# mbrzus/Cross-Modality-Minipig-Gan

Hardware: NVIDIA B200
Metric: gan_train_image_pairs_per_sec (higher is better)
Workload: dtype bf16

## Files before the change

### cross-modality-minipig-gan_b200/csrc/conv_c1mma.cuh

```cuda
#pragma once

namespace mpgan {
namespace tc {

constexpr int kC1Threads = 512;
constexpr int kC1XStages = 16;
constexpr int kC1XBytes = 2304;
constexpr int kC1Stages = 8;
constexpr int kC1StageBytes = 128 * 32;

struct C1mmaParams {
  int nimg, ih, iw, oh, ow, stride, pad;
  int tiles_w, tiles_h, total_tiles;
  int xrow;
  uint32_t xbytes;
  int xoff;
  int wide;
  const bf16* w;
  bf16* out;
  long long out_sn, out_sh, out_sw;
  const float* bias;
  double* stats;
};

template <int N>
__global__ void __launch_bounds__(kC1Threads, 1)
c1mma_fprop_kernel(const __grid_constant__ C1mmaParams P, const __grid_constant__ CUtensorMap tmX) {
  constexpr int NACC = 512 / N > 8 ? 8 : 512 / N;
  constexpr int TMEM_COLS = NACC * N < 32 ? 32 : NACC * N;
  constexpr int CH = N >= 32 ? 32 : 16;
  constexpr int NCH = N / CH;
  constexpr uint32_t kEmptyArrivals = NCH == 1 ? 4u : 8u;
  extern __shared__ __align__(1024) uint8_t smem[];
  if ((smem_u32(smem) & 1023u) != 0) __trap();
  uint8_t* a_sm = smem;
  uint8_t* x_sm = smem + kC1Stages * kC1StageBytes;
  uint8_t* w_sm = x_sm + kC1XStages * kC1XBytes;
  uint64_t* a_full = reinterpret_cast<uint64_t*>(w_sm + 2048);
  uint64_t* a_empty = a_full + kC1Stages;
  uint64_t* tfull = a_empty + kC1Stages;
  uint64_t* tempty = tfull + 8;
  uint64_t* x_full = tempty + 8;
  uint64_t* x_empty = x_full + kC1XStages;
  uint32_t* tmem_slot = reinterpret_cast<uint32_t*>(x_empty + kC1XStages);
  float* s_stats = reinterpret_cast<float*>(w_sm + 2048 + 1024);
  float* s_bias = s_stats + 8 * 2 * N;

  const int warp = threadIdx.x >> 5, lane = threadIdx.x & 31;
  if (threadIdx.x == 0) {
    for (int i = 0; i < kC1Stages; ++i) { mbar_init(&a_full[i], 1); mbar_init(&a_empty[i], 1); }
    for (int i = 0; i < 8; ++i) { mbar_init(&tfull[i], 1); mbar_init(&tempty[i], kEmptyArrivals); }
    for (int i = 0; i < kC1XStages; ++i) { mbar_init(&x_full[i], 1); mbar_init(&x_empty[i], 1); }
    fence_barrier_init();
    prefetch_tmap(&tmX);
  }
  if (warp == 4) tmem_alloc<TMEM_COLS>(tmem_slot);
  for (int i = threadIdx.x; i < 8 * 2 * N; i += blockDim.x) s_stats[i] = 0.f;
  pdl_wait();
  pdl_launch();
  if (threadIdx.x < N) {
    const int n = threadIdx.x;
    uint32_t v[8];
#pragma unroll
    for (int j = 0; j < 8; ++j) v[j] = 0u;
#pragma unroll
    for (int t = 0; t < 9; ++t) {
      const uint32_t b = (uint32_t)__bfloat16_as_ushort(P.w[n * 9 + t]);
      v[t >> 1] |= (t & 1) ? (b << 16) : b;
    }
    const uint32_t sw = (uint32_t)(n >> 2) & 1u;
    *reinterpret_cast<uint4*>(w_sm + n * 32 + ((0u ^ sw) << 4)) = make_uint4(v[0], v[1], v[2], v[3]);
    *reinterpret_cast<uint4*>(w_sm + n * 32 + ((1u ^ sw) << 4)) = make_uint4(v[4], v[5], v[6], v[7]);
    s_bias[n] = P.bias ? __ldg(&P.bias[n]) : 0.f;
    asm volatile("fence.proxy.async.shared::cta;" ::: "memory");
  }
  tc_fence_before();
  __syncthreads();
  tc_fence_after();
  const uint32_t tmem_base = *tmem_slot;
  const int tiles_per_img = P.tiles_w * P.tiles_h;

  if (warp == 5) {
    if (elect_one()) {
      int xs = 0;
      uint32_t xpar = 0;
      TileWalk<3> tw;
      { const int radix[3] = {P.tiles_w, P.tiles_h, 1 << 30}; tw.init((int)blockIdx.x, (int)gridDim.x, radix); }
      for (int tile = blockIdx.x; tile < P.total_tiles; tile += gridDim.x, tw.next()) {
        const int twi = tw.d[0], thi = tw.d[1], img = tw.d[2];
        mbar_wait(&x_empty[xs], xpar ^ 1);
        mbar_expect_tx(&x_full[xs], P.xbytes);
        tma_load_3d(x_sm + xs * kC1XBytes, &tmX, &x_full[xs], twi * HT_W * P.stride - P.pad - P.xoff,
                    thi * HT_H * P.stride - P.pad, img);
        if (++xs == kC1XStages) { xs = 0; xpar ^= 1; }
      }
    }
  } else if (warp < 4) {
    const int S = P.stride;
    int it = warp;
    for (int tile = blockIdx.x + warp * gridDim.x; tile < P.total_tiles; tile += 4 * gridDim.x, it += 4) {
      const int stage = it % kC1Stages;
      const uint32_t par = (uint32_t)(it / kC1Stages) & 1u;
      const int xs = it % kC1XStages;
      const uint32_t xpar = (uint32_t)(it / kC1XStages) & 1u;
      mbar_wait(&x_full[xs], xpar);
      const uint8_t* xw = x_sm + xs * kC1XBytes;
      uint32_t v[4][9];
#pragma unroll
      for (int k = 0; k < 4; ++k) {
// ... 54 lines not shown
    for (int j = 0; j < CH / 2; ++j) { s1[j] = 0ull; s2[j] = 0ull; }
    int it = 0;
    TileWalk<3> tw;
    { const int radix[3] = {P.tiles_w, P.tiles_h, 1 << 30}; tw.init((int)blockIdx.x, (int)gridDim.x, radix); }
    for (int tile = blockIdx.x; tile < P.total_tiles; tile += gridDim.x, ++it, tw.next()) {
      if (NCH == 1 && (it & 1) != half) continue;
      const int twi = tw.d[0], thi = tw.d[1], img = tw.d[2];
      const int oh = thi * HT_H + lh, ow = twi * HT_W + lw;
      const bool valid = oh < P.oh && ow < P.ow;
      bf16* orow = P.out + (long long)img * P.out_sn + (long long)oh * P.out_sh + (long long)ow * P.out_sw + c0;
      const int acc = it % NACC;
      const uint32_t par = (uint32_t)(it / NACC) & 1u;
      mbar_wait(&tfull[acc], par);
      tc_fence_after();
      const uint32_t t_addr = tmem_base + ((uint32_t)(q * 32) << 16) + (uint32_t)(acc * N + c0);
      uint32_t r[CH];
      if (CH == 32) tmem_ld_32x32(t_addr, r);
      else tmem_ld_32x16(t_addr, r);
      tmem_ld_wait();
      tc_fence_before();
      __syncwarp();
      if (lane == 0) mbar_arrive(&tempty[acc]);
      epi_chunk_store<CH>(r, s_bias + c0, orow, valid, P.stats != nullptr, s1, s2, nullptr, P.wide != 0);
    }
    if (P.stats) {
      float v[32];
#pragma unroll
      for (int j = 0; j < 32; ++j) v[j] = j < CH ? ((j & 1) ? unpack_f32x2(s1[j / 2]).y : unpack_f32x2(s1[j / 2]).x) : 0.f;
      const float t1 = warp_transpose_reduce32(v, lane);
#pragma unroll
      for (int j = 0; j < 32; ++j) v[j] = j < CH ? ((j & 1) ? unpack_f32x2(s2[j / 2]).y : unpack_f32x2(s2[j / 2]).x) : 0.f;
      const float t2 = warp_transpose_reduce32(v, lane);
      if (lane < CH) { sl[c0 + lane] = t1; sl[N + c0 + lane] = t2; }
    }
  }
  __syncwarp();
  tc_fence_before();
  __syncthreads();
  if (P.stats) {
    for (int i = threadIdx.x; i < 2 * N; i += blockDim.x) {
      double s = 0.0;
#pragma unroll
      for (int e = 0; e < 8; ++e) s += (double)s_stats[e * 2 * N + i];
      if (s != 0.0) atomicAdd(&P.stats[i], s);
    }
  }
  if (warp == 4) {
    tc_fence_after();
    tmem_dealloc<TMEM_COLS>(tmem_base);
  }
}

template <int N>
static int launch_c1mma(const C1mmaParams& P, const CUtensorMap& mX, cudaStream_t s) {
  const size_t smem = (size_t)kC1Stages * kC1StageBytes + (size_t)kC1XStages * kC1XBytes + 2048 + 1024 +
                      (size_t)8 * 2 * N * 4 + (size_t)N * 4 + 64;
  static bool attr_done = false;
  if (!attr_done) {
    cudaError_t e = cudaFuncSetAttribute(c1mma_fprop_kernel<N>, cudaFuncAttributeMaxDynamicSharedMemorySize, 96 * 1024);
    MPGAN_REQUIRE(e == cudaSuccess, MPGAN_ERR_CUDA, "cudaFuncSetAttribute(c1mma): %s", cudaGetErrorString(e));
    attr_done = true;
  }
  const int grid = P.total_tiles < num_sms() ? P.total_tiles : num_sms();
  launch_k(c1mma_fprop_kernel<N>, grid, kC1Threads, smem, s, P, mX);
  MPGAN_CHECK_LAUNCH("c1mma_fprop_kernel");
  return 0;
}

}

int c1mma_fprop(const MpganConvGeom* g, int dtype, const void* x, int64_t ldx, const void* w, const float* bias, void* y,
                int64_t ldy, double* stats, cudaStream_t s) {
  using namespace tc;
  if (!g || dtype != MPGAN_BF16 || g->rank != 2 || g->cx != 1) return 1;
  if (g->k[1] != 3 || g->k[2] != 3 || g->stride[1] != g->stride[2] || (g->stride[1] != 1 && g->stride[1] != 2)) return 1;
  if (g->pad[1] != g->pad[2] || g->pad[1] < 0 || g->pad[1] > 1) return 1;
  if (g->stride[1] != 1) return 1;
  const int N = g->cy;
  if (!(N == 16 || N == 32 || N == 64)) return 1;
  if (ldy % 8 != 0 || ((uintptr_t)y & 15) || ((uintptr_t)x & 15)) return 1;
  if (ldx != 1 || g->xs[2] % 8 != 0) return 1;
  C1mmaParams P;
  memset(&P, 0, sizeof(P));
  P.nimg = g->n; P.ih = g->xs[1]; P.iw = g->xs[2]; P.oh = g->ys[1]; P.ow = g->ys[2];
  P.stride = g->stride[1]; P.pad = g->pad[1];
  P.tiles_w = (P.ow + HT_W - 1) / HT_W; P.tiles_h = (P.oh + HT_H - 1) / HT_H;
  P.total_tiles = g->n * P.tiles_w * P.tiles_h;
  P.w = (const bf16*)w;
  P.xoff = P.pad ? 8 - P.pad : 0;
  const int need = (HT_W - 1) * P.stride + 3 + P.xoff;
  const int bw = need <= 16 ? 16 : 32, bh = (HT_H - 1) * P.stride + 3;
  P.xrow = bw * 2; P.xbytes = (uint32_t)(bw * 2 * bh);
  if ((int)P.xbytes > kC1XBytes) return 1;
  CUtensorMap mX;
  {
    uint64_t dims[3] = {(uint64_t)P.iw, (uint64_t)P.ih, (uint64_t)g->n};
    uint64_t str[2] = {(uint64_t)P.iw, (uint64_t)P.iw * P.ih};
    uint32_t box[3] = {(uint32_t)bw, (uint32_t)bh, 1u};
    int rc = encode_map(&mX, x, 3, dims, str, box, true);
    if (rc) return rc;
  }
  P.out = (bf16*)y;
  P.out_sn = (long long)P.oh * P.ow * ldy; P.out_sh = (long long)P.ow * ldy; P.out_sw = ldy;
  P.bias = bias; P.stats = stats;
  P.wide = (ldy % 16 == 0 && ((uintptr_t)y & 31) == 0) ? 1 : 0;
  switch (N) {
    case 16: return launch_c1mma<16>(P, mX, s);
    case 32: return launch_c1mma<32>(P, mX, s);
    default: return launch_c1mma<64>(P, mX, s);
  }
}

}
```

### cross-modality-minipig-gan_b200/csrc/conv_tc.cu

```cuda
#include <cudaTypedefs.h>
#include <algorithm>
#include <stdlib.h>
#include <string.h>

#include "common.cuh"
#include "tc_common.cuh"

namespace mpgan {
namespace tc {

constexpr int MAXT = 64;
constexpr int MAXCLS = 8;
constexpr int kSmemLimit = 227 * 1024;

struct ActMaps { CUtensorMap m[8]; };

struct TapGemmParams {
  int ncls;
  int cls_tap_begin[MAXCLS + 1];
  int cls_od[MAXCLS], cls_oh[MAXCLS], cls_ow[MAXCLS];
  long long cls_out_off[MAXCLS];
  signed char tap_map[MAXT];
  short tap_dd[MAXT], tap_dh[MAXT], tap_dw[MAXT], tap_slab[MAXT];
  int nkc;
// ... 1137 lines not shown
}

extern "C" size_t mpgan_tc_conv_wgrad_workspace(const MpganConvGeom* g) {
  (void)g;
  return 0;
}

extern "C" int mpgan_tc_conv_wgrad(const MpganConvGeom* g, const void* x, int64_t ldx, const void* y, int64_t ldy,
                                   float* dw, void* workspace, size_t workspace_bytes, void* stream) {
  (void)workspace; (void)workspace_bytes;
  Geom2 g2;
  int rc = to_geom2(g, &g2);
  if (rc) return rc;
  return run_wgrad(g2, x, ldx, y, ldy, dw, (cudaStream_t)stream);
}
```

### cross-modality-minipig-gan_b200/mpgan/_lib.py

```python
import ctypes
import os
import re
from ctypes import c_char_p, c_double, c_float, c_int, c_int32, c_int64, c_size_t, c_void_p, POINTER, Structure

_HERE = os.path.dirname(os.path.abspath(__file__))
LIB_PATH = os.path.join(os.path.dirname(_HERE), "libmpgan_sm100.so")
HEADER_PATH = os.path.join(os.path.dirname(os.path.dirname(_HERE)), "include", "mpgan.h")

F32, BF16 = 0, 1
ACT_NONE, ACT_PRELU, ACT_LEAKY, ACT_TANH = 0, 1, 2, 3


class ConvGeom(Structure):
    _fields_ = [("rank", c_int32), ("n", c_int32), ("xs", c_int32 * 3), ("ys", c_int32 * 3), ("cx", c_int32),
                ("cy", c_int32), ("k", c_int32 * 3), ("stride", c_int32 * 3), ("pad", c_int32 * 3)]


_G = POINTER(ConvGeom)
_P = c_void_p
_SIGS = {
    "mpgan_version": (c_int, []),
    "mpgan_last_error": (c_char_p, []),
    "mpgan_device_ok": (c_int, []),
    "mpgan_conv_fprop": (c_int, [_G, c_int, _P, c_int64, _P, _P, _P, c_int64, _P]),
# ... 36 lines not shown
    "mpgan_bce_bwd": (c_int, [_P, _P, c_float, _P, _P, c_int32, _P]),
    "mpgan_l1_fwd": (c_int, [c_int, _P, _P, c_int64, c_float, _P, _P]),
    "mpgan_l1_bwd": (c_int, [c_int, _P, _P, c_int64, c_float, _P, _P, c_int, _P]),
    "mpgan_l1_fwd_bwd": (c_int, [c_int, _P, _P, c_int64, c_float, _P, _P, _P, _P, c_int, _P]),
    "mpgan_adam_step": (c_int, [_P, _P, _P, _P, c_int64, c_float, c_float, c_float, c_float, _P, _P, _P]),
    "mpgan_cast": (c_int, [c_int, _P, c_int, _P, c_int64, _P]),
    "mpgan_weight_transpose": (c_int, [c_int, _P, c_int, _P, c_int32, c_int32, c_int32, _P]),
    "mpgan_weight_transpose_batch": (c_int, [_P, c_int32, c_int32, _P]),
    "mpgan_patch_gather": (c_int, [c_int, _P, c_int32, c_int32, _P, c_int32, _P, c_int32, c_int32, _P, _P]),
    "mpgan_patch_scatter_add": (c_int, [c_int, _P, c_int32, c_int32, _P, c_int32, _P, c_int32, c_int32, _P, _P]),
    "mpgan_c1_tail_fwd": (c_int, [_P, c_int32, c_int32, c_int32, _P, _P, _P, c_float, c_float, _P, _P, _P, _P, _P, _P,
                                  _P, _P, _P, _P, _P, _P, _P]),
    "mpgan_c1_tail_bwd_reduce": (c_int, [_P, _P, c_int32, c_int32, c_int32, _P, _P, _P, _P, _P, _P, _P, _P, _P]),
    "mpgan_im2col_c1": (c_int, [_P, c_int32, c_int32, c_int32, c_int32, c_int32, c_int32, c_int32, _P, _P]),
    "mpgan_fold_dw16": (c_int, [_P, c_int32, _P, _P]),
    "mpgan_im2col_c1_vol": (c_int, [_P, c_int32, POINTER(c_int32), POINTER(c_int32), c_int32, c_int32, _P, _P]),
    "mpgan_col2im_c1_vol": (c_int, [_P, c_int32, POINTER(c_int32), POINTER(c_int32), c_int32, c_int32, _P, _P, _P, _P]),
    "mpgan_fold_dw32": (c_int, [_P, c_int32, _P, _P]),
    "mpgan_stencil27": (c_int, [c_int, c_int, _P, c_int32, c_int32, c_int32, c_int32, _P, _P, _P, _P, _P]),
    "mpgan_stencil27_wgrad": (c_int, [c_int, _P, _P, c_int32, c_int32, c_int32, c_int32, _P, _P, _P]),
    "mpgan_order_stats_workspace": (c_size_t, [c_int32]),
    "mpgan_order_stats": (c_int, [_P, c_int64, _P, c_int32, _P, _P, c_size_t, _P]),
    "mpgan_minmax": (c_int, [_P, c_int64, _P, c_int32, _P, _P, c_size_t, _P]),
    "mpgan_rescale_intensity": (c_int, [_P, c_int64, c_float, c_float, c_float, c_float, c_int, c_float, c_float, c_int,
                                        c_int, _P, _P]),
    "mpgan_err_sums": (c_int, [_P, _P, c_int64, _P, _P]),
    "mpgan_ssim_sums": (c_int, [_P, _P, c_int32, c_int32, c_int32, c_int32, c_int32, POINTER(c_double), c_int32, c_double,
                                c_double, c_double, _P, _P]),
    "mpgan_mutual_info_workspace": (c_size_t, [c_int32]),
    "mpgan_mutual_info": (c_int, [_P, _P, c_int32, c_int64, c_int32, _P, _P, _P, _P, c_size_t, _P]),
# ... 50 lines not shown
```

### cross-modality-minipig-gan_b200/mpgan/nets.py

```python
import os

import numpy as np
import torch
import torch.nn as nn

from . import ops
from ._lib import ACT_LEAKY, ACT_NONE, ACT_PRELU
from .runtime import Runtime

_CONV = {2: nn.Conv2d, 3: nn.Conv3d}
_CONVT = {2: nn.ConvTranspose2d, 3: nn.ConvTranspose3d}
_BN = {2: nn.BatchNorm2d, 3: nn.BatchNorm3d}

DEFAULT_PRECISION = "bf16"


def remap_monai_keys(state_dict, to="legacy"):
    out = type(state_dict)() if isinstance(state_dict, dict) else {}
    for k, v in state_dict.items():
        if to == "legacy":
            k = k.replace(".adn.N.", ".norm.").replace(".adn.A.", ".act.")
        elif "generator." in k or k.startswith("model."):
            k = k.replace(".norm.", ".adn.N.").replace(".act.", ".adn.A.")
        out[k] = v
# ... 539 lines not shown
        self._init_runtime(precision)

    def _run(self, x, save, want_acts, need_wgrad=None, logical_acts=True):
        rt = self.runtime
        rt.ensure(x.device)
        plan = Plan(rt, self.training, save, rt.requires_grad() if need_wgrad is None else need_wgrad)
        xin = self._to_cl(x.float())
        h = ops.add_copy(xin, None, _new(xin, xin.shape, rt.dtype)) if rt.dtype != torch.float32 else xin
        acts = []
        convs = [m for m in self.model_conv if isinstance(m, (nn.Conv2d, nn.Conv3d))]
        bns = [m for m in self.model_conv if isinstance(m, (nn.BatchNorm2d, nn.BatchNorm3d))]
        for conv, bn in zip(convs, bns):
            rec = rt.rec[conv]
            ch = conv.out_channels
            stats = plan.zeros64(2 * ch, x.device) if plan.training else None
            c, fused = conv_apply(rec, h, stats=stats)
            if want_acts:
                bn_out, saved = bn_act_forward(c, bn, ACT_NONE, None, 0.0, None, None, plan, stats, fused)
                y = ops.bn_act_apply(bn_out, None, None, ACT_LEAKY, None, 0.2, None, _new(c, c.shape))
                acts += [("sp", c), ("sp", bn_out), ("sp", y)]
            else:
                bn_out = None
                y, saved = bn_act_forward(c, bn, ACT_LEAKY, None, 0.2, None, None, plan, stats, fused)
            if save:
                plan.tape.append((h, c, saved, plan.training, bn_out))
            h = y
        n = h.shape[0]
        feat_shape = tuple(h.shape)
        hf = h.reshape(n, -1)
        if want_acts:
# ... 94 lines not shown
            nd = self.dims
            g = g.permute((0,) + tuple(range(2, nd + 2)) + (1,)).reshape(dfeat.shape)
            dfeat = dfeat + g.to(dfeat.dtype)
        dh = dfeat.reshape(feat_shape)
        convs = [m for m in self.model_conv if isinstance(m, (nn.Conv2d, nn.Conv3d))]
        bns = [m for m in self.model_conv if isinstance(m, (nn.BatchNorm2d, nn.BatchNorm3d))]
        nd = self.dims
        to_cl = (0,) + tuple(range(2, nd + 2)) + (1,)
        for i in range(len(convs) - 1, -1, -1):
            h_in, c, saved, trained, bn_out = plan.tape.pop()
            if (3 * i + 2) in ag:
                if internal:
                    dh = inject(dh.contiguous(), ag[3 * i + 2])
                else:
                    dh = dh + ag[3 * i + 2].permute(to_cl).to(dh.dtype)
            if bn_out is not None:
                dbn = ops.act_bwd(dh.contiguous(), bn_out, ACT_LEAKY, 0.2, _new(bn_out, bn_out.shape))
                if (3 * i + 1) in ag:
                    dbn = inject(dbn, ag[3 * i + 1]) if internal else dbn + ag[3 * i + 1].permute(to_cl).to(dbn.dtype)
                dc = bn_act_backward(dbn, c, saved, bns[i], ACT_NONE, None, 0.0, plan, trained)
                fused_bias = False
            else:
                fused_bias = (3 * i) not in ag
                dc = bn_act_backward(dh, c, saved, bns[i], ACT_LEAKY, None, 0.2, plan, trained,
                                     conv_db=rt.rec[convs[i]].db if fused_bias else None)
            if (3 * i) in ag:
                dc = inject(dc, ag[3 * i]) if internal else dc + ag[3 * i].permute(to_cl).to(dc.dtype)
            dh = conv_backward(rt.rec[convs[i]], h_in, dc, plan, need_dx=(need_dx or i > 0), bias_done=fused_bias)
            if on_layer_done is not None:
                forked = plan.wgrad_forked and N_WGRAD_STREAMS == 1
                if plan.wgrad_forked and not forked:
# ... 46 lines not shown
```

### cross-modality-minipig-gan_b200/mpgan/ops.py

```python
import bisect
import ctypes
import os

import torch

from . import _lib
from ._lib import ACT_LEAKY, ACT_NONE, ACT_PRELU, ACT_TANH, BF16, F32, ConvGeom, check

_NULL = None


def _stream():
    return torch.cuda.current_stream().cuda_stream


def dt(t):
    if t.dtype == torch.float32:
        return F32
    if t.dtype == torch.bfloat16:
        return BF16
    raise TypeError(f"unsupported dtype {t.dtype}")


def ptr(t):
# ... 266 lines not shown
        g1 = _spec_1x1(16, spec.cy).geom(n, ys, ys)
        check(lib.mpgan_tc_conv_wgrad(ctypes.byref(g1), ptr(xcol), 16, ptr(y), ld(y), ptr(dw16), None, 0, _stream()),
              "tc_conv_wgrad(im2col)")
        check(lib.mpgan_fold_dw16(ptr(dw16), spec.cy, ptr(dw), _stream()), "fold_dw16")
    elif use_tc and x.dtype == torch.bfloat16 and tc_supported(g, 2):
        check(lib.mpgan_tc_conv_wgrad(ctypes.byref(g), ptr(x), ld(x), ptr(y), ld(y), ptr(dw), None, 0, _stream()),
              "tc_conv_wgrad")
    elif use_c1 and lib.mpgan_c1_supported(ctypes.byref(g), 2):
        check(lib.mpgan_c1_conv_wgrad(ctypes.byref(g), dt(x), ptr(x), ld(x), ptr(y), ld(y), ptr(dw), _stream()),
              "c1_conv_wgrad")
    else:
        check(lib.mpgan_conv_wgrad(ctypes.byref(g), dt(x), ptr(x), ld(x), ptr(y), ld(y), ptr(dw), _stream()),
              "conv_wgrad")


def colsum(x, out):
    lib = _lib.require_device()
    check(lib.mpgan_colsum(dt(x), ptr(x), ld(x), pixels(x), x.shape[-1], ptr(out), _stream()), "colsum")


def bn_stats(x, stats):
    lib = _lib.require_device()
    check(lib.mpgan_bn_stats(dt(x), ptr(x), ld(x), pixels(x), x.shape[-1], ptr(stats), _stream()), "bn_stats")


def bn_finalize(stats, npix, bn, training, mean, invstd, scale, shift):
    lib = _lib.require_device()
    mom = 0.1 if bn.momentum is None else bn.momentum
    check(lib.mpgan_bn_finalize(ptr(stats), npix, bn.num_features, ptr(bn.weight), ptr(bn.bias), bn.eps, mom,
                                1 if training else 0, ptr(bn.running_mean), ptr(bn.running_var),
# ... 328 lines not shown
```

### include/mpgan.h

```cpp
#ifndef MPGAN_H_
#define MPGAN_H_

#include <stddef.h>
#include <stdint.h>

#ifdef __cplusplus
extern "C" {
#endif

#define MPGAN_VERSION 100

enum { MPGAN_OK = 0, MPGAN_ERR_SHAPE = -1, MPGAN_ERR_UNSUPPORTED = -2, MPGAN_ERR_CUDA = -3 };
enum { MPGAN_F32 = 0, MPGAN_BF16 = 1 };
enum { MPGAN_ACT_NONE = 0, MPGAN_ACT_PRELU = 1, MPGAN_ACT_LEAKY = 2, MPGAN_ACT_TANH = 3 };

typedef struct {
  int32_t rank;
  int32_t n;
  int32_t xs[3];
  int32_t ys[3];
  int32_t cx, cy;
  int32_t k[3], stride[3], pad[3];
} MpganConvGeom;

// ... 98 lines not shown
                            void* stream);

int mpgan_c1_tail_fwd(const void* c_bf16, int32_t n, int32_t h, int32_t w, const double* stats, const float* gamma,
                      const float* beta, float eps, float momentum, float* running_mean, float* running_var,
                      int64_t* num_batches_tracked, float* mean, float* invstd, float* scale, float* shift,
                      const float* alpha, const void* w9_bf16, const float* bias, void* h_out_bf16, void* y_out_bf16,
                      void* stream);
int mpgan_c1_tail_bwd_reduce(const void* dy_bf16, const void* c_bf16, int32_t n, int32_t h, int32_t w, const float* mean,
                             const float* invstd, const float* scale, const float* shift, const float* alpha,
                             const void* w9_bf16, void* dh_bf16, double* sums3, void* stream);

int mpgan_im2col_c1(const void* x_bf16, int32_t n, int32_t ih, int32_t iw, int32_t oh, int32_t ow, int32_t stride,
                    int32_t pad, void* xcol_bf16, void* stream);
int mpgan_fold_dw16(const float* dw16, int32_t cy, float* dw, void* stream);

int mpgan_im2col_c1_vol(const void* x_bf16, int32_t n, const int32_t* xs3, const int32_t* ys3, int32_t stride, int32_t pad,
                        void* xcol_bf16, void* stream);
int mpgan_col2im_c1_vol(const void* t_bf16, int32_t n, const int32_t* xs3, const int32_t* ys3, int32_t stride, int32_t pad,
                        const float* bias, const void* res_bf16, void* x_bf16, void* stream);
int mpgan_fold_dw32(const float* dw32, int32_t cy, float* dw, void* stream);
int mpgan_stencil27(int dtype, int direction, const void* in, int32_t n, int32_t d, int32_t h, int32_t w, const void* w27,
                    const float* bias, const void* res, void* out, void* stream);
int mpgan_stencil27_wgrad(int dtype, const void* x, const void* dy, int32_t n, int32_t d, int32_t h, int32_t w, float* dw27,
                          float* dbias, void* stream);

size_t mpgan_order_stats_workspace(int32_t nranks);
int mpgan_order_stats(const float* x, int64_t n, const int64_t* ranks, int32_t nranks, float* out, void* workspace,
                      size_t workspace_bytes, void* stream);
int mpgan_minmax(const float* x, int64_t n, const int64_t* ranks, int32_t nranks, float* out, void* workspace,
                 size_t workspace_bytes, void* stream);
// ... 23 lines not shown
```

Measured before the change: 1755.

## Fuse discriminator layer-1 conv with BatchNorm and LeakyReLU via recompute

Adds BatchNorm-aware modes to the 1-channel 3x3 tensor-core conv kernel. The forward pass runs the conv twice, once for statistics only and once applying BN plus LeakyReLU, so the large 64-channel pre-activation tensor is never written. Backward recomputes the conv, streams dy through a new TMA producer warp, and fuses the BN/activation gradient reduction and apply into two passes. This trades extra cheap conv recompute and larger shared-memory use for avoiding reads and writes of the full-resolution intermediate activations.

```diff
diff --git a/cross-modality-minipig-gan_b200/csrc/conv_c1mma.cuh b/cross-modality-minipig-gan_b200/csrc/conv_c1mma.cuh
--- a/cross-modality-minipig-gan_b200/csrc/conv_c1mma.cuh
+++ b/cross-modality-minipig-gan_b200/csrc/conv_c1mma.cuh
@@ -8,6 +8,14 @@
 constexpr int kC1XBytes = 2304;
 constexpr int kC1Stages = 8;
 constexpr int kC1StageBytes = 128 * 32;
+constexpr int kC1DyStages = 8;
+constexpr int kC1DyBytes = 128 * 64 * 2;
+
+enum { C1_CONV = 0,
+       C1_STATS = 1,
+       C1_FWD = 2,
+       C1_REDUCE = 3,
+       C1_APPLY = 4 };
 
 struct C1mmaParams {
   int nimg, ih, iw, oh, ow, stride, pad;
@@ -21,11 +29,127 @@
   long long out_sn, out_sh, out_sw;
   const float* bias;
   double* stats;
+  long long npix;
+  float slope;
+  const double* stats_in;
+  const float* gamma; const float* beta; float eps, momentum;
+  float* running_mean; float* running_var; long long* nbt;
+  float* mean; float* invstd; float* scale; float* shift;
+  float* dgamma; float* dbeta; float* dbias;
 };
 
-template <int N>
+__host__ __device__ constexpr int c1_dy_offset(int N) {
+  return (kC1Stages * kC1StageBytes + kC1XStages * kC1XBytes + 2048 + 1024 + 8 * 2 * N * 4 + N * 4 + 4 * N * 4 + 1023) &
+         ~1023;
+}
+
+template <int MODE>
+__device__ __forceinline__ void c1_bn_coef(const C1mmaParams& P, int n, int N, float* s_coef) {
+  if (MODE == C1_FWD) {
+    const double m = P.stats_in[n] / (double)P.npix;
+    double var = P.stats_in[N + n] / (double)P.npix - m * m;
+    if (var < 0.0) var = 0.0;
+    const float mean = (float)m;
+    const float invstd = (float)(1.0 / sqrt(var + (double)P.eps));
+    const float g = P.gamma ? P.gamma[n] : 1.f, b = P.beta ? P.beta[n] : 0.f;
+    const float sc = g * invstd;
+    const float sh = b - mean * sc;
+    if (blockIdx.x == 0) {
+      if (P.running_mean) P.running_mean[n] = (1.f - P.momentum) * P.running_mean[n] + P.momentum * mean;
+      if (P.running_var) {
+        const double unb = P.npix > 1 ? var * ((double)P.npix / (double)(P.npix - 1)) : var;
+        P.running_var[n] = (1.f - P.momentum) * P.running_var[n] + P.momentum * (float)unb;
+      }
+      P.mean[n] = mean; P.invstd[n] = invstd; P.scale[n] = sc; P.shift[n] = sh;
+      if (n == 0 && P.nbt) *P.nbt += 1;
+    }
+    s_coef[n] = sc; s_coef[N + n] = sh;
+  } else if (MODE == C1_REDUCE) {
+    const float sc = P.scale[n], sh = P.shift[n], mu = P.mean[n], is = P.invstd[n];
+    s_coef[n] = sc; s_coef[N + n] = sh; s_coef[2 * N + n] = is; s_coef[3 * N + n] = -mu * is;
+  } else if (MODE == C1_APPLY) {
+    const float invP = 1.f / (float)P.npix;
+    const float sc = P.scale[n], sh = P.shift[n], mu = P.mean[n], is = P.invstd[n];
+    const float mg = (float)P.stats_in[n] * invP;
+    const float mgx = (float)P.stats_in[N + n] * invP;
+    const float k2 = -sc * is * mgx;
+    s_coef[n] = sc; s_coef[N + n] = sh; s_coef[2 * N + n] = k2; s_coef[3 * N + n] = -sc * mg - k2 * mu;
+    if (blockIdx.x == 0) {
+      if (P.dbeta) P.dbeta[n] += (float)P.stats_in[n];
+      if (P.dgamma) P.dgamma[n] += (float)P.stats_in[N + n];
+    }
+  }
+}
+
+template <int MODE>
+__device__ __forceinline__ void c1_bn_epilogue(const uint32_t (&r)[16], int hh, const float* s_bias_c0, const float* s_coef_c0,
+                                               const uint8_t* dyrow, int rsw, int chunk0, bf16* orow, bool valid,
+                                               float slope, unsigned long long (&s1)[16], unsigned long long (&s2)[16]) {
+  constexpr int N = 64;
+  const unsigned long long ones = pack_f32x2(1.f, 1.f);
+  s_bias_c0 += 16 * hh; s_coef_c0 += 16 * hh; chunk0 += 2 * hh; orow += 16 * hh;
+  uint32_t o[8];
+  uint4 gq = make_uint4(0u, 0u, 0u, 0u);
+#pragma unroll
+  for (int j = 0; j < 8; ++j) {
+    const int js = 8 * hh + j;
+    if ((MODE == C1_REDUCE || MODE == C1_APPLY) && (j & 3) == 0)
+      gq = *reinterpret_cast<const uint4*>(dyrow + (((chunk0 + (j >> 2)) ^ rsw) << 4));
+    const float2 b = *reinterpret_cast<const float2*>(s_bias_c0 + 2 * j);
+    const float2 v = unpack_f32x2(fma_f32x2(pack_f32x2(__uint_as_float(r[2 * j]), __uint_as_float(r[2 * j + 1])), ones,
+                                            pack_f32x2(b.x, b.y)));
+    __nv_bfloat162 h = __floats2bfloat162_rn(v.x, v.y);
+    const uint32_t hc = *reinterpret_cast<uint32_t*>(&h);
+    const unsigned long long c = pack_f32x2(__uint_as_float(hc << 16), __uint_as_float(hc & 0xffff0000u));
+    if (MODE == C1_STATS) {
+      if (valid) {
+        s1[js] = fma_f32x2(c, ones, s1[js]);
+        s2[js] = fma_f32x2(c, c, s2[js]);
+      }
+      continue;
+    }
+    const float2 sc = *reinterpret_cast<const float2*>(s_coef_c0 + 2 * j);
+    const float2 sh = *reinterpret_cast<const float2*>(s_coef_c0 + N + 2 * j);
+    const float2 z = unpack_f32x2(fma_f32x2(c, pack_f32x2(sc.x, sc.y), pack_f32x2(sh.x, sh.y)));
+    if (MODE == C1_FWD) {
+      const float yx = z.x > 0.f ? z.x : z.x * slope, yy = z.y > 0.f ? z.y : z.y * slope;
+      __nv_bfloat162 hy = __floats2bfloat162_rn(yx, yy);
+      o[j] = *reinterpret_cast<uint32_t*>(&hy);
+      continue;
+    }
+    const float2 kc = *reinterpret_cast<const float2*>(s_coef_c0 + 2 * N + 2 * j);
+    const float2 kd = *reinterpret_cast<const float2*>(s_coef_c0 + 3 * N + 2 * j);
+    const uint32_t gw = (j & 3) == 0 ? gq.x : (j & 3) == 1 ? gq.y : (j & 3) == 2 ? gq.z : gq.w;
+    const float gx = __uint_as_float(gw << 16), gy = __uint_as_float(gw & 0xffff0000u);
+    const float2 gz = make_float2(gx * (z.x > 0.f ? 1.f : slope), gy * (z.y > 0.f ? 1.f : slope));
+    if (MODE == C1_REDUCE) {
+      const unsigned long long xh = fma_f32x2(c, pack_f32x2(kc.x, kc.y), pack_f32x2(kd.x, kd.y));
+      if (valid) {
+        const float2 a = unpack_f32x2(s1[js]);
+        s1[js] = pack_f32x2(a.x + gz.x, a.y + gz.y);
+        s2[js] = fma_f32x2(pack_f32x2(gz.x, gz.y), xh, s2[js]);
+      }
+    } else {
+      const float2 dx = unpack_f32x2(fma_f32x2(pack_f32x2(sc.x, sc.y), pack_f32x2(gz.x, gz.y),
+                                               fma_f32x2(pack_f32x2(kc.x, kc.y), c, pack_f32x2(kd.x, kd.y))));
+      __nv_bfloat162 hd = __floats2bfloat162_rn(dx.x, dx.y);
+      o[j] = *reinterpret_cast<uint32_t*>(&hd);
+      if (valid) {
+        const float2 a = unpack_f32x2(s1[js]);
+        s1[js] = pack_f32x2(a.x + __uint_as_float(o[j] << 16), a.y + __uint_as_float(o[j] & 0xffff0000u));
+      }
+    }
+  }
+  if ((MODE == C1_FWD || MODE == C1_APPLY) && valid)
+    st_global_256(orow, o[0], o[1], o[2], o[3], o[4], o[5], o[6], o[7]);
+}
+
+template <int N, int MODE>
 __global__ void __launch_bounds__(kC1Threads, 1)
-c1mma_fprop_kernel(const __grid_constant__ C1mmaParams P, const __grid_constant__ CUtensorMap tmX) {
+c1mma_fprop_kernel(const __grid_constant__ C1mmaParams P, const __grid_constant__ CUtensorMap tmX,
+                   const __grid_constant__ CUtensorMap tmDy) {
+  static_assert(MODE == C1_CONV || N == 64, "the BatchNorm modes are D layer 1 (64 channels)");
+  constexpr bool kDy = MODE == C1_REDUCE || MODE == C1_APPLY;
   constexpr int NACC = 512 / N > 8 ? 8 : 512 / N;
   constexpr int TMEM_COLS = NACC * N < 32 ? 32 : NACC * N;
   constexpr int CH = N >= 32 ? 32 : 16;
@@ -42,17 +166,24 @@
   uint64_t* tempty = tfull + 8;
   uint64_t* x_full = tempty + 8;
   uint64_t* x_empty = x_full + kC1XStages;
-  uint32_t* tmem_slot = reinterpret_cast<uint32_t*>(x_empty + kC1XStages);
+  uint64_t* dy_full = x_empty + kC1XStages;
+  uint64_t* dy_empty = dy_full + kC1DyStages;
+  uint32_t* tmem_slot = reinterpret_cast<uint32_t*>(dy_empty + kC1DyStages);
   float* s_stats = reinterpret_cast<float*>(w_sm + 2048 + 1024);
   float* s_bias = s_stats + 8 * 2 * N;
+  float* s_coef = s_bias + N;
+  uint8_t* dy_sm = smem + c1_dy_offset(N);
 
   const int warp = threadIdx.x >> 5, lane = threadIdx.x & 31;
   if (threadIdx.x == 0) {
     for (int i = 0; i < kC1Stages; ++i) { mbar_init(&a_full[i], 1); mbar_init(&a_empty[i], 1); }
     for (int i = 0; i < 8; ++i) { mbar_init(&tfull[i], 1); mbar_init(&tempty[i], kEmptyArrivals); }
     for (int i = 0; i < kC1XStages; ++i) { mbar_init(&x_full[i], 1); mbar_init(&x_empty[i], 1); }
+    if (kDy)
+      for (int i = 0; i < kC1DyStages; ++i) { mbar_init(&dy_full[i], 1); mbar_init(&dy_empty[i], 8); }
     fence_barrier_init();
     prefetch_tmap(&tmX);
+    if (kDy) prefetch_tmap(&tmDy);
   }
   if (warp == 4) tmem_alloc<TMEM_COLS>(tmem_slot);
   for (int i = threadIdx.x; i < 8 * 2 * N; i += blockDim.x) s_stats[i] = 0.f;
@@ -73,6 +204,7 @@
     *reinterpret_cast<uint4*>(w_sm + n * 32 + ((1u ^ sw) << 4)) = make_uint4(v[4], v[5], v[6], v[7]);
     s_bias[n] = P.bias ? __ldg(&P.bias[n]) : 0.f;
     asm volatile("fence.proxy.async.shared::cta;" ::: "memory");
+    if (MODE != C1_CONV && MODE != C1_STATS) c1_bn_coef<MODE>(P, n, N, s_coef);
   }
   tc_fence_before();
   __syncthreads();
@@ -93,6 +225,19 @@
         tma_load_3d(x_sm + xs * kC1XBytes, &tmX, &x_full[xs], twi * HT_W * P.stride - P.pad - P.xoff,
                     thi * HT_H * P.stride - P.pad, img);
         if (++xs == kC1XStages) { xs = 0; xpar ^= 1; }
+      }
+    }
+  } else if (warp == 6) {
+    if (kDy && elect_one()) {
+      int ds = 0;
+      uint32_t dpar = 0;
+      TileWalk<3> tw;
+      { const int radix[3] = {P.tiles_w, P.tiles_h, 1 << 30}; tw.init((int)blockIdx.x, (int)gridDim.x, radix); }
+      for (int tile = blockIdx.x; tile < P.total_tiles; tile += gridDim.x, tw.next()) {
+        mbar_wait(&dy_empty[ds], dpar ^ 1);
+        mbar_expect_tx(&dy_full[ds], (uint32_t)kC1DyBytes);
+        tma_load_4d(dy_sm + ds * kC1DyBytes, &tmDy, &dy_full[ds], 0, tw.d[0] * HT_W, tw.d[1] * HT_H, tw.d[2]);
+        if (++ds == kC1DyStages) { ds = 0; dpar ^= 1; }
       }
     }
   } else if (warp < 4) {
@@ -177,16 +322,54 @@
       mbar_wait(&tfull[acc], par);
       tc_fence_after();
       const uint32_t t_addr = tmem_base + ((uint32_t)(q * 32) << 16) + (uint32_t)(acc * N + c0);
-      uint32_t r[CH];
-      if (CH == 32) tmem_ld_32x32(t_addr, r);
-      else tmem_ld_32x16(t_addr, r);
-      tmem_ld_wait();
-      tc_fence_before();
-      __syncwarp();
-      if (lane == 0) mbar_arrive(&tempty[acc]);
-      epi_chunk_store<CH>(r, s_bias + c0, orow, valid, P.stats != nullptr, s1, s2, nullptr, P.wide != 0);
-    }
-    if (P.stats) {
+      if constexpr (MODE == C1_CONV) {
+        uint32_t r[CH];
+        if (CH == 32) tmem_ld_32x32(t_addr, r);
+        else tmem_ld_32x16(t_addr, r);
+        tmem_ld_wait();
+        tc_fence_before();
+        __syncwarp();
+        if (lane == 0) mbar_arrive(&tempty[acc]);
+        epi_chunk_store<CH>(r, s_bias + c0, orow, valid, P.stats != nullptr, s1, s2, nullptr, P.wide != 0);
+      } else {
+        const uint8_t* dyrow = nullptr;
+        int ds = 0;
+        if (kDy) {
+          ds = it % kC1DyStages;
+          mbar_wait(&dy_full[ds], (uint32_t)(it / kC1DyStages) & 1u);
+          dyrow = dy_sm + ds * kC1DyBytes + row * 128;
+        }
+#pragma unroll
+        for (int hh = 0; hh < 2; ++hh) {
+          uint32_t r[16];
+          tmem_ld_32x16(t_addr + 16 * hh, r);
+          tmem_ld_wait();
+          if (hh == 1) {
+            tc_fence_before();
+            __syncwarp();
+            if (lane == 0) mbar_arrive(&tempty[acc]);
+          }
+          c1_bn_epilogue<MODE>(r, hh, s_bias + c0, s_coef + c0, dyrow, row & 7, c0 / 8, orow, valid, P.slope, s1, s2);
+        }
+        if (kDy) {
+          __syncwarp();
+          if (lane == 0) mbar_arrive(&dy_empty[ds]);
+        }
+      }
+    }
+    if (MODE != C1_CONV && MODE != C1_FWD) {
+      float v[32];
+#pragma unroll
+      for (int j = 0; j < 32; ++j) v[j] = (j & 1) ? unpack_f32x2(s1[j / 2]).y : unpack_f32x2(s1[j / 2]).x;
+      const float t1 = warp_transpose_reduce32(v, lane);
+      float t2 = 0.f;
+      if (MODE != C1_APPLY) {
+#pragma unroll
+        for (int j = 0; j < 32; ++j) v[j] = (j & 1) ? unpack_f32x2(s2[j / 2]).y : unpack_f32x2(s2[j / 2]).x;
+        t2 = warp_transpose_reduce32(v, lane);
+      }
+      sl[c0 + lane] = t1; sl[N + c0 + lane] = t2;
+    } else if (MODE == C1_CONV && P.stats) {
       float v[32];
 #pragma unroll
       for (int j = 0; j < 32; ++j) v[j] = j < CH ? ((j & 1) ? unpack_f32x2(s1[j / 2]).y : unpack_f32x2(s1[j / 2]).x) : 0.f;
@@ -200,7 +383,15 @@
   __syncwarp();
   tc_fence_before();
   __syncthreads();
-  if (P.stats) {
+  if (MODE == C1_APPLY) {
+    if (P.dbias)
+      for (int i = threadIdx.x; i < N; i += blockDim.x) {
+        double s = 0.0;
+#pragma unroll
+        for (int e = 0; e < 8; ++e) s += (double)s_stats[e * 2 * N + i];
+        atomicAdd(&P.dbias[i], (float)s);
+      }
+  } else if (MODE != C1_FWD && P.stats) {
     for (int i = threadIdx.x; i < 2 * N; i += blockDim.x) {
       double s = 0.0;
 #pragma unroll
@@ -214,26 +405,29 @@
   }
 }
 
-template <int N>
-static int launch_c1mma(const C1mmaParams& P, const CUtensorMap& mX, cudaStream_t s) {
-  const size_t smem = (size_t)kC1Stages * kC1StageBytes + (size_t)kC1XStages * kC1XBytes + 2048 + 1024 +
-                      (size_t)8 * 2 * N * 4 + (size_t)N * 4 + 64;
+template <int N, int MODE>
+static int launch_c1mma(const C1mmaParams& P, const CUtensorMap& mX, const CUtensorMap& mDy, cudaStream_t s) {
+  size_t smem = (size_t)kC1Stages * kC1StageBytes + (size_t)kC1XStages * kC1XBytes + 2048 + 1024 +
+                (size_t)8 * 2 * N * 4 + (size_t)N * 4 + 64;
+  if (MODE != C1_CONV) smem += (size_t)4 * N * 4;
+  if (MODE == C1_REDUCE || MODE == C1_APPLY) smem = (size_t)c1_dy_offset(N) + (size_t)kC1DyStages * kC1DyBytes + 64;
   static bool attr_done = false;
   if (!attr_done) {
-    cudaError_t e = cudaFuncSetAttribute(c1mma_fprop_kernel<N>, cudaFuncAttributeMaxDynamicSharedMemorySize, 96 * 1024);
+    cudaError_t e = cudaFuncSetAttribute(c1mma_fprop_kernel<N, MODE>, cudaFuncAttributeMaxDynamicSharedMemorySize,
+                                         (int)(smem > 96 * 1024 ? kSmemLimit : 96 * 1024));
     MPGAN_REQUIRE(e == cudaSuccess, MPGAN_ERR_CUDA, "cudaFuncSetAttribute(c1mma): %s", cudaGetErrorString(e));
     attr_done = true;
   }
   const int grid = P.total_tiles < num_sms() ? P.total_tiles : num_sms();
-  launch_k(c1mma_fprop_kernel<N>, grid, kC1Threads, smem, s, P, mX);
+  launch_k(c1mma_fprop_kernel<N, MODE>, grid, kC1Threads, smem, s, P, mX, mDy);
   MPGAN_CHECK_LAUNCH("c1mma_fprop_kernel");
   return 0;
 }
 
 }
 
-int c1mma_fprop(const MpganConvGeom* g, int dtype, const void* x, int64_t ldx, const void* w, const float* bias, void* y,
-                int64_t ldy, double* stats, cudaStream_t s) {
+static int c1mma_setup(const MpganConvGeom* g, int dtype, const void* x, int64_t ldx, const void* w, const float* bias,
+                       tc::C1mmaParams* P, CUtensorMap* mX) {
   using namespace tc;
   if (!g || dtype != MPGAN_BF16 || g->rank != 2 || g->cx != 1) return 1;
   if (g->k[1] != 3 || g->k[2] != 3 || g->stride[1] != g->stride[2] || (g->stride[1] != 1 && g->stride[1] != 2)) return 1;
@@ -241,37 +435,80 @@
   if (g->stride[1] != 1) return 1;
   const int N = g->cy;
   if (!(N == 16 || N == 32 || N == 64)) return 1;
-  if (ldy % 8 != 0 || ((uintptr_t)y & 15) || ((uintptr_t)x & 15)) return 1;
+  if ((uintptr_t)x & 15) return 1;
   if (ldx != 1 || g->xs[2] % 8 != 0) return 1;
+  memset(P, 0, sizeof(*P));
+  P->nimg = g->n; P->ih = g->xs[1]; P->iw = g->xs[2]; P->oh = g->ys[1]; P->ow = g->ys[2];
+  P->stride = g->stride[1]; P->pad = g->pad[1];
+  P->tiles_w = (P->ow + HT_W - 1) / HT_W; P->tiles_h = (P->oh + HT_H - 1) / HT_H;
+  P->total_tiles = g->n * P->tiles_w * P->tiles_h;
+  P->w = (const bf16*)w;
+  P->bias = bias;
+  P->npix = (long long)g->n * P->oh * P->ow;
+  P->xoff = P->pad ? 8 - P->pad : 0;
+  const int need = (HT_W - 1) * P->stride + 3 + P->xoff;
+  const int bw = need <= 16 ? 16 : 32, bh = (HT_H - 1) * P->stride + 3;
+  P->xrow = bw * 2; P->xbytes = (uint32_t)(bw * 2 * bh);
+  if ((int)P->xbytes > kC1XBytes) return 1;
+  uint64_t dims[3] = {(uint64_t)P->iw, (uint64_t)P->ih, (uint64_t)g->n};
+  uint64_t str[2] = {(uint64_t)P->iw, (uint64_t)P->iw * P->ih};
+  uint32_t box[3] = {(uint32_t)bw, (uint32_t)bh, 1u};
+  return encode_map(mX, x, 3, dims, str, box, true);
+}
+
+int c1mma_fprop(const MpganConvGeom* g, int dtype, const void* x, int64_t ldx, const void* w, const float* bias, void* y,
+                int64_t ldy, double* stats, cudaStream_t s) {
+  using namespace tc;
   C1mmaParams P;
-  memset(&P, 0, sizeof(P));
-  P.nimg = g->n; P.ih = g->xs[1]; P.iw = g->xs[2]; P.oh = g->ys[1]; P.ow = g->ys[2];
-  P.stride = g->stride[1]; P.pad = g->pad[1];
-  P.tiles_w = (P.ow + HT_W - 1) / HT_W; P.tiles_h = (P.oh + HT_H - 1) / HT_H;
-  P.total_tiles = g->n * P.tiles_w * P.tiles_h;
-  P.w = (const bf16*)w;
-  P.xoff = P.pad ? 8 - P.pad : 0;
-  const int need = (HT_W - 1) * P.stride + 3 + P.xoff;
-  const int bw = need <= 16 ? 16 : 32, bh = (HT_H - 1) * P.stride + 3;
-  P.xrow = bw * 2; P.xbytes = (uint32_t)(bw * 2 * bh);
-  if ((int)P.xbytes > kC1XBytes) return 1;
   CUtensorMap mX;
-  {
-    uint64_t dims[3] = {(uint64_t)P.iw, (uint64_t)P.ih, (uint64_t)g->n};
-    uint64_t str[2] = {(uint64_t)P.iw, (uint64_t)P.iw * P.ih};
-    uint32_t box[3] = {(uint32_t)bw, (uint32_t)bh, 1u};
-    int rc = encode_map(&mX, x, 3, dims, str, box, true);
-    if (rc) return rc;
-  }
+  if (ldy % 8 != 0 || ((uintptr_t)y & 15)) return 1;
+  int rc = c1mma_setup(g, dtype, x, ldx, w, bias, &P, &mX);
+  if (rc) return rc;
   P.out = (bf16*)y;
   P.out_sn = (long long)P.oh * P.ow * ldy; P.out_sh = (long long)P.ow * ldy; P.out_sw = ldy;
-  P.bias = bias; P.stats = stats;
+  P.stats = stats;
   P.wide = (ldy % 16 == 0 && ((uintptr_t)y & 31) == 0) ? 1 : 0;
-  switch (N) {
-    case 16: return launch_c1mma<16>(P, mX, s);
-    case 32: return launch_c1mma<32>(P, mX, s);
-    default: return launch_c1mma<64>(P, mX, s);
-  }
-}
-
-}
+  switch (g->cy) {
+    case 16: return launch_c1mma<16, C1_CONV>(P, mX, mX, s);
+    case 32: return launch_c1mma<32, C1_CONV>(P, mX, mX, s);
+    default: return launch_c1mma<64, C1_CONV>(P, mX, mX, s);
+  }
+}
+
+static int c1bn_run(int mode, const MpganConvGeom* g, const void* x, const void* w, const float* bias, tc::C1mmaParams& P,
+                    const void* dy, void* out, cudaStream_t s) {
+  using namespace tc;
+  const tc::C1mmaParams keep = P;
+  CUtensorMap mX, mDy;
+  MPGAN_REQUIRE(g && g->cy == 64 && g->pad[1] == 0, MPGAN_ERR_UNSUPPORTED, "c1bn: 64 output channels, no padding");
+  int rc = c1mma_setup(g, MPGAN_BF16, x, 1, w, bias, &P, &mX);
+  MPGAN_REQUIRE(rc != 1, MPGAN_ERR_UNSUPPORTED, "c1bn: layer not covered by the one-channel tcgen05 kernel");
+  if (rc) return rc;
+  P.stats = keep.stats; P.slope = keep.slope; P.stats_in = keep.stats_in;
+  P.gamma = keep.gamma; P.beta = keep.beta; P.eps = keep.eps; P.momentum = keep.momentum;
+  P.running_mean = keep.running_mean; P.running_var = keep.running_var; P.nbt = keep.nbt;
+  P.mean = keep.mean; P.invstd = keep.invstd; P.scale = keep.scale; P.shift = keep.shift;
+  P.dgamma = keep.dgamma; P.dbeta = keep.dbeta; P.dbias = keep.dbias;
+  if (out) {
+    MPGAN_REQUIRE(((uintptr_t)out & 31) == 0, MPGAN_ERR_SHAPE, "c1bn: output not 32-byte aligned");
+    P.out = (bf16*)out;
+    P.out_sn = (long long)P.oh * P.ow * 64; P.out_sh = (long long)P.ow * 64; P.out_sw = 64;
+    P.wide = 1;
+  }
+  mDy = mX;
+  if (dy) {
+    uint64_t dims[4] = {64u, (uint64_t)P.ow, (uint64_t)P.oh, (uint64_t)g->n};
+    uint64_t str[3] = {64u, (uint64_t)P.ow * 64, (uint64_t)P.ow * P.oh * 64};
+    uint32_t box[4] = {64u, (uint32_t)HT_W, (uint32_t)HT_H, 1u};
+    rc = encode_map(&mDy, dy, 4, dims, str, box);
+    if (rc) return rc;
+  }
+  switch (mode) {
+    case C1_STATS: return launch_c1mma<64, C1_STATS>(P, mX, mDy, s);
+    case C1_FWD: return launch_c1mma<64, C1_FWD>(P, mX, mDy, s);
+    case C1_REDUCE: return launch_c1mma<64, C1_REDUCE>(P, mX, mDy, s);
+    default: return launch_c1mma<64, C1_APPLY>(P, mX, mDy, s);
+  }
+}
+
+}
diff --git a/cross-modality-minipig-gan_b200/csrc/conv_tc.cu b/cross-modality-minipig-gan_b200/csrc/conv_tc.cu
--- a/cross-modality-minipig-gan_b200/csrc/conv_tc.cu
+++ b/cross-modality-minipig-gan_b200/csrc/conv_tc.cu
@@ -1175,3 +1175,39 @@
   if (rc) return rc;
   return run_wgrad(g2, x, ldx, y, ldy, dw, (cudaStream_t)stream);
 }
+
+
+extern "C" int mpgan_c1bn_fwd(const MpganConvGeom* g, const void* x, const void* w, const float* bias, double* stats,
+                              const float* gamma, const float* beta, float eps, float momentum, float* running_mean,
+                              float* running_var, int64_t* num_batches_tracked, float* mean, float* invstd, float* scale,
+                              float* shift, float leaky_slope, void* y, void* stream) {
+  MPGAN_REQUIRE(stats && mean && invstd && scale && shift && y, MPGAN_ERR_SHAPE, "c1bn_fwd: bad arguments");
+  tc::C1mmaParams P;
+  memset(&P, 0, sizeof(P));
+  P.stats = stats;
+  int rc = c1bn_run(tc::C1_STATS, g, x, w, bias, P, nullptr, nullptr, (cudaStream_t)stream);
+  if (rc) return rc;
+  memset(&P, 0, sizeof(P));
+  P.stats_in = stats; P.gamma = gamma; P.beta = beta; P.eps = eps; P.momentum = momentum;
+  P.running_mean = running_mean; P.running_var = running_var; P.nbt = (long long*)num_batches_tracked;
+  P.mean = mean; P.invstd = invstd; P.scale = scale; P.shift = shift; P.slope = leaky_slope;
+  return c1bn_run(tc::C1_FWD, g, x, w, bias, P, nullptr, y, (cudaStream_t)stream);
+}
+
+extern "C" int mpgan_c1bn_bwd(const MpganConvGeom* g, const void* x, const void* w, const float* bias, const void* dy,
+                              const float* mean, const float* invstd, const float* scale, const float* shift,
+                              float leaky_slope, double* sums, float* dgamma, float* dbeta, float* dbias, void* dc,
+                              void* stream) {
+  MPGAN_REQUIRE(dy && mean && invstd && scale && shift && sums && dc, MPGAN_ERR_SHAPE, "c1bn_bwd: bad arguments");
+  tc::C1mmaParams P;
+  memset(&P, 0, sizeof(P));
+  P.mean = const_cast<float*>(mean); P.invstd = const_cast<float*>(invstd);
+  P.scale = const_cast<float*>(scale); P.shift = const_cast<float*>(shift);
+  P.slope = leaky_slope;
+  P.stats = sums;
+  int rc = c1bn_run(tc::C1_REDUCE, g, x, w, bias, P, dy, nullptr, (cudaStream_t)stream);
+  if (rc) return rc;
+  P.stats = nullptr;
+  P.stats_in = sums; P.dgamma = dgamma; P.dbeta = dbeta; P.dbias = dbias;
+  return c1bn_run(tc::C1_APPLY, g, x, w, bias, P, dy, dc, (cudaStream_t)stream);
+}
diff --git a/cross-modality-minipig-gan_b200/mpgan/_lib.py b/cross-modality-minipig-gan_b200/mpgan/_lib.py
--- a/cross-modality-minipig-gan_b200/mpgan/_lib.py
+++ b/cross-modality-minipig-gan_b200/mpgan/_lib.py
@@ -74,6 +74,8 @@
     "mpgan_c1_tail_bwd_reduce": (c_int, [_P, _P, c_int32, c_int32, c_int32, _P, _P, _P, _P, _P, _P, _P, _P, _P]),
     "mpgan_im2col_c1": (c_int, [_P, c_int32, c_int32, c_int32, c_int32, c_int32, c_int32, c_int32, _P, _P]),
     "mpgan_fold_dw16": (c_int, [_P, c_int32, _P, _P]),
+    "mpgan_c1bn_fwd": (c_int, [_G, _P, _P, _P, _P, _P, _P, c_float, c_float, _P, _P, _P, _P, _P, _P, _P, c_float, _P, _P]),
+    "mpgan_c1bn_bwd": (c_int, [_G, _P, _P, _P, _P, _P, _P, _P, _P, c_float, _P, _P, _P, _P, _P, _P]),
     "mpgan_im2col_c1_vol": (c_int, [_P, c_int32, POINTER(c_int32), POINTER(c_int32), c_int32, c_int32, _P, _P]),
     "mpgan_col2im_c1_vol": (c_int, [_P, c_int32, POINTER(c_int32), POINTER(c_int32), c_int32, c_int32, _P, _P, _P, _P]),
     "mpgan_fold_dw32": (c_int, [_P, c_int32, _P, _P]),
diff --git a/cross-modality-minipig-gan_b200/mpgan/nets.py b/cross-modality-minipig-gan_b200/mpgan/nets.py
--- a/cross-modality-minipig-gan_b200/mpgan/nets.py
+++ b/cross-modality-minipig-gan_b200/mpgan/nets.py
@@ -577,6 +577,14 @@
             rec = rt.rec[conv]
             ch = conv.out_channels
             stats = plan.zeros64(2 * ch, x.device) if plan.training else None
+            if plan.training and not want_acts and ops.c1bn_ok(rec.spec, h):
+                saved = torch.empty((4, ch), dtype=torch.float32, device=x.device)
+                y = ops.c1bn_fwd(rec.spec, h, rec.w, rec.bias, stats, bn, saved, 0.2)
+                rt.bn_version += 1
+                if save:
+                    plan.tape.append((h, None, saved, True, None))
+                h = y
+                continue
             c, fused = conv_apply(rec, h, stats=stats)
             if want_acts:
                 bn_out, saved = bn_act_forward(c, bn, ACT_NONE, None, 0.0, None, None, plan, stats, fused)
@@ -701,7 +709,14 @@
                     dh = inject(dh.contiguous(), ag[3 * i + 2])
                 else:
                     dh = dh + ag[3 * i + 2].permute(to_cl).to(dh.dtype)
-            if bn_out is not None:
+            if c is None:
+                rec = rt.rec[convs[i]]
+                wg = plan.need_wgrad
+                dc = ops.c1bn_bwd(rec.spec, h_in, rec.w, rec.bias, dh, saved, 0.2,
+                                  plan.zeros64(2 * rec.spec.cy + 1, dh.device), bns[i].weight.grad if wg else None,
+                                  bns[i].bias.grad if wg else None, rec.db if wg else None)
+                fused_bias = True
+            elif bn_out is not None:
                 dbn = ops.act_bwd(dh.contiguous(), bn_out, ACT_LEAKY, 0.2, _new(bn_out, bn_out.shape))
                 if (3 * i + 1) in ag:
                     dbn = inject(dbn, ag[3 * i + 1]) if internal else dbn + ag[3 * i + 1].permute(to_cl).to(dbn.dtype)
diff --git a/cross-modality-minipig-gan_b200/mpgan/ops.py b/cross-modality-minipig-gan_b200/mpgan/ops.py
--- a/cross-modality-minipig-gan_b200/mpgan/ops.py
+++ b/cross-modality-minipig-gan_b200/mpgan/ops.py
@@ -304,6 +304,48 @@
               "conv_wgrad")
 
 
+_D1FUSE = os.environ.get("MPGAN_NO_D1FUSE", "0") != "1"
+
+
+def c1bn_ok(spec, x, force=False):
+    if not (_D1FUSE and x.dtype == torch.bfloat16 and spec.rank == 2 and not spec.transposed and spec.cx == 1
+            and spec.cy == 64 and spec.k == (3, 3) and spec.stride == (1, 1) and spec.pad == (0, 0)
+            and x.is_contiguous() and x.shape[2] % 8 == 0 and x.data_ptr() % 16 == 0):
+        return False
+    ys = spec.y_of_x(tuple(x.shape[1:-1]))
+    return force or x.shape[0] * ys[0] * ys[1] > (1 << 20)
+
+
+def c1bn_fwd(spec, x, w, bias, stats, bn, saved, leaky, out=None):
+    lib = _lib.require_device()
+    n, xs = x.shape[0], tuple(x.shape[1:-1])
+    ys = spec.y_of_x(xs)
+    if out is None:
+        out = torch.empty((n,) + ys + (spec.cy,), dtype=x.dtype, device=x.device)
+    assert out.is_contiguous() and out.dtype == torch.bfloat16
+    mom = 0.1 if bn.momentum is None else bn.momentum
+    g = spec.geom(n, xs, ys)
+    check(lib.mpgan_c1bn_fwd(ctypes.byref(g), ptr(x), ptr(w), ptr(bias), ptr(stats), ptr(bn.weight), ptr(bn.bias), bn.eps,
+                             mom, ptr(bn.running_mean), ptr(bn.running_var), ptr(bn.num_batches_tracked), ptr(saved[0]),
+                             ptr(saved[1]), ptr(saved[2]), ptr(saved[3]), leaky, ptr(out), _stream()), "c1bn_fwd")
+    return out
+
+
+def c1bn_bwd(spec, x, w, bias, dy, saved, leaky, sums, dgamma, dbeta, dbias, dc=None):
+    lib = _lib.require_device()
+    n, xs = x.shape[0], tuple(x.shape[1:-1])
+    ys = spec.y_of_x(xs)
+    dy = dy.contiguous()
+    if dc is None:
+        dc = torch.empty_like(dy)
+    assert dc.is_contiguous() and dy.shape == (n,) + ys + (spec.cy,)
+    g = spec.geom(n, xs, ys)
+    check(lib.mpgan_c1bn_bwd(ctypes.byref(g), ptr(x), ptr(w), ptr(bias), ptr(dy), ptr(saved[0]), ptr(saved[1]),
+                             ptr(saved[2]), ptr(saved[3]), leaky, ptr(sums), ptr(dgamma), ptr(dbeta), ptr(dbias), ptr(dc),
+                             _stream()), "c1bn_bwd")
+    return dc
+
+
 def colsum(x, out):
     lib = _lib.require_device()
     check(lib.mpgan_colsum(dt(x), ptr(x), ld(x), pixels(x), x.shape[-1], ptr(out), _stream()), "colsum")
diff --git a/include/mpgan.h b/include/mpgan.h
--- a/include/mpgan.h
+++ b/include/mpgan.h
@@ -136,6 +136,14 @@
                     int32_t pad, void* xcol_bf16, void* stream);
 int mpgan_fold_dw16(const float* dw16, int32_t cy, float* dw, void* stream);
 
+int mpgan_c1bn_fwd(const MpganConvGeom* g, const void* x, const void* w, const float* bias, double* stats,
+                   const float* gamma, const float* beta, float eps, float momentum, float* running_mean,
+                   float* running_var, int64_t* num_batches_tracked, float* mean, float* invstd, float* scale,
+                   float* shift, float leaky_slope, void* y, void* stream);
+int mpgan_c1bn_bwd(const MpganConvGeom* g, const void* x, const void* w, const float* bias, const void* dy,
+                   const float* mean, const float* invstd, const float* scale, const float* shift, float leaky_slope,
+                   double* sums, float* dgamma, float* dbeta, float* dbias, void* dc, void* stream);
+
 int mpgan_im2col_c1_vol(const void* x_bf16, int32_t n, const int32_t* xs3, const int32_t* ys3, int32_t stride, int32_t pad,
                         void* xcol_bf16, void* stream);
 int mpgan_col2im_c1_vol(const void* t_bf16, int32_t n, const int32_t* xs3, const int32_t* ys3, int32_t stride, int32_t pad,
```

Measured after the change: 1765 (median of 6 runs). No clear change (+0.6%).
